# microsoft/esvit

Measured on NVIDIA H100. Metric: multi-crop images/sec, Swin-T W7 pretrain step (2 global 224^2 + 8 local 96^2 crops, DDINOLoss V+R, K=65536), higher is better.
Workload: dtype bf16

## Files before the change

### esvit_b200/_lib.py

```python
from __future__ import annotations

import ctypes
import os
from ctypes import c_double, c_float, c_int, c_longlong, c_void_p

HERE = os.path.dirname(os.path.abspath(__file__))
LIB_PATH = os.path.join(HERE, "lib", "libesvit_b200.so")
HEADER_PATH = os.path.join(os.path.dirname(HERE), "include", "esvit_b200.h")

ERR_BAD_ARG = 1001

P, I, L, F, D = c_void_p, c_int, c_longlong, c_float, c_double

SIGNATURES = {
    "esvit_add_ln_fwd": [P, P, P, I, P, P, F, P, P, I, P, P, L, I, P],
    "esvit_add_ln_bwd": [P, I, P, P, P, P, P, P, I, P, P, P, P, P, L, I, P],
    "esvit_patch_merge_ln_fwd": [P, P, P, F, P, P, P, I, I, I, I, P],
    "esvit_patch_merge_ln_bwd": [P, P, P, P, P, P, P, P, I, I, I, I, P],
    "esvit_token_mean_fwd": [P, P, I, I, I, P],
    "esvit_token_mean_bwd": [P, P, P, I, I, I, P],
    "esvit_patch_embed_fwd": [P, P, P, P, P, F, P, P, P, I, I, I, I, P],
    "esvit_patch_embed_bwd": [P, P, P, P, P, P, P, P, P, P, P, I, I, I, I, P],
    "esvit_window_attn_expand_bias": [P, P, I, I, P],
    "esvit_window_attn_fwd": [P, P, P, P, I, P, P, I, I, I, I, I, I, I, F, P],
    "esvit_window_attn_bwd": [P, P, P, P, I, P, P, P, P, P, P, I, I, I, I, I, I, I, F, P],
    "esvit_window_attn_probs": [P, P, P, P, I, P, I, I, I, I, I, I, I, F, P],
    "esvit_gemm_bias_act": [P, P, P, P, P, L, I, I, I, P],
    "esvit_gemm_mul_colsum": [P, P, P, P, P, P, L, I, I, P],
    "esvit_gemm_bf16": [P, P, P, P, P, L, I, I, I, I, I, I, P],
    "esvit_gemm_mul_colsum2": [P, P, P, P, P, P, L, I, I, I, I, P],
    "esvit_gemm_wgrad_ws_floats": [I, I],
    "esvit_gemm_wgrad": [P, P, P, P, L, I, I, I, I, P],
    "esvit_gelu_fwd": [P, P, L, P],
    "esvit_gelu_bwd": [P, P, P, L, P],
    "esvit_gelu_bwd_dbias": [P, P, P, P, L, I, P],
    "esvit_mul_bwd_dbias": [P, P, P, P, L, I, P],
    "esvit_l2norm_fwd": [P, P, P, F, L, I, P],
    "esvit_l2norm_bwd": [P, P, P, P, L, I, P],
    "esvit_weight_norm_fwd": [P, P, P, P, L, I, P],
    "esvit_weight_norm_bwd": [P, P, P, P, I, P, P, L, I, P],
    "esvit_row_lse": [P, P, F, P, L, I, P],
    "esvit_dino_ce_fwd": [P, P, P, P, P, P, P, F, F, P, L, I, P],
    "esvit_dino_ce_bwd": [P, P, P, P, P, P, P, P, P, F, F, P, L, I, P],
    "esvit_weighted_sum": [P, P, I, P, P],
    "esvit_row_softmax_q_max_k": [],
    "esvit_row_softmax_q": [P, P, F, P, P, L, I, P],
    "esvit_dino_ce_q_fwd": [P, P, P, P, P, F, P, L, I, P],
    "esvit_dino_ce_q_bwd": [P, P, P, P, P, P, P, F, P, L, I, P],
    "esvit_colsum_workspace_rows": [],
    "esvit_colsum": [P, L, I, P, P, P],
    "esvit_center_ema": [P, P, F, F, P, I, P],
    "esvit_normalize_rows": [P, P, L, I, F, P],
    "esvit_region_match": [P, P, I, I, I, I, I, P, P, P],
    "esvit_mhsa_fwd": [P, P, P, I, I, I, I, F, P],
    "esvit_mhsa_bwd": [P, P, P, P, P, P, I, I, I, I, F, P],
    "esvit_vit_patches": [P, P, I, I, I, P],
    "esvit_vit_tokens_fwd": [P, P, P, P, I, I, I, P],
    "esvit_vit_tokens_bwd": [P, P, P, P, P, I, I, I, I, P],
    "esvit_vit_split": [P, P, P, I, I, I, I, P],
    "esvit_ema_multi": [P, P, P, I, D, P],
    "esvit_clip_multi": [P, P, I, F, P, P, P],
    "esvit_grad_sumsq_multi": [P, P, I, P, P],
    "esvit_adamw_ema_multi": [P, P, P, P, P, P, P, P, I, P, P, P, P],
    "esvit_knn_prep": [P, P, P, P, L, L, I, P],
    "esvit_knn_select": [P, L, P, P, P, P, P, I, I, I, I, I, P, P, P, P, P, P],
# ... 29 lines not shown

def _cuda_error_string(code: int) -> str:
    try:
        import torch
        return torch.cuda.cudart().cudaGetErrorString(code) if hasattr(torch.cuda.cudart(), "cudaGetErrorString") \
            else f"cudaError {code}"
    except Exception:
        return f"cudaError {code}"


def call(name: str, *args) -> None:
    rc = getattr(load(), name)(*args)
    if rc != 0:
        if rc == ERR_BAD_ARG:
            raise ValueError(f"{name}: unsupported shape / argument (ESVIT_ERR_BAD_ARG)")
        raise EsvitKernelError(f"{name} failed: {_cuda_error_string(rc)} (status {rc})")


_LAUNCHES = {"esvit_colsum": 2, "esvit_gemm_mul_colsum": 2, "esvit_gemm_mul_colsum2": 2, "esvit_gemm_wgrad": 2}
_launch_count = 0
_timed_names = set()
_timed_events = []
_META = {
    "esvit_dino_ce_bwd": lambda a: {"rows": int(a[-3]), "K": int(a[-2])},
    "esvit_window_attn_bwd": lambda a: _attn_meta(a),
    "esvit_window_attn_fwd": lambda a: _attn_meta(a),
    "esvit_window_attn_probs": lambda a: _attn_meta(a),
    "esvit_gemm_bias_act": lambda a: {"M": int(a[5]), "N": int(a[6]), "K": int(a[7])},
    "esvit_gemm_mul_colsum": lambda a: {"M": int(a[6]), "N": int(a[7]), "K": int(a[8])},
    "esvit_gemm_bf16": lambda a: {"M": int(a[5]), "N": int(a[6]), "K": int(a[7]), "b_mn": int(a[9]), "act": int(a[10]),
                                  "pre": a[4] is not None and a[4].value is not None},
    "esvit_gemm_mul_colsum2": lambda a: {"M": int(a[6]), "N": int(a[7]), "K": int(a[8])},
    "esvit_gemm_wgrad": lambda a: {"T": int(a[4]), "N": int(a[5]), "K": int(a[6])},
    "esvit_add_ln_fwd": lambda a: {"T": int(a[-3]), "C": int(a[-2]), "has_x": a[0] is not None and a[0].value is not None,
                                   "has_delta": a[1] is not None and a[1].value is not None},
    "esvit_add_ln_bwd": lambda a: {"T": int(a[-3]), "C": int(a[-2])},
    "esvit_dino_ce_fwd": lambda a: {"rows": int(a[-3]), "K": int(a[-2])},
    "esvit_dino_ce_q_fwd": lambda a: {"rows": int(a[-3]), "K": int(a[-2])},
    "esvit_dino_ce_q_bwd": lambda a: {"rows": int(a[-3]), "K": int(a[-2])},
    "esvit_row_softmax_q": lambda a: {"rows": int(a[-3]), "K": int(a[-2])},
    "esvit_mhsa_fwd": lambda a: {"B": int(a[3]), "L": int(a[4]), "C": int(a[5]), "nH": int(a[6])},
    "esvit_mhsa_bwd": lambda a: {"B": int(a[6]), "L": int(a[7]), "C": int(a[8]), "nH": int(a[9])},
    "esvit_vit_tokens_bwd": lambda a: {"B": int(a[-5]), "N": int(a[-4]), "D": int(a[-3])},
    "esvit_patch_embed_fwd": lambda a: {"B": int(a[-5]), "H": int(a[-4]), "W": int(a[-3]), "E": int(a[-2])},
    "esvit_patch_embed_bwd": lambda a: {"B": int(a[-5]), "H": int(a[-4]), "W": int(a[-3]), "E": int(a[-2])},
}


def _attn_meta(a):
    B, H, W, C, nH, ws = (int(a[i]) for i in (-9, -8, -7, -6, -5, -4))
    return {"tokens": B * H * W, "C": C, "nH": nH, "ws": ws, "windows": B * (-(-H // ws)) * (-(-W // ws))}


def reset_counters() -> None:
    global _launch_count
    _launch_count = 0
    _timed_events.clear()


def launch_count() -> int:
    return _launch_count


def time_entry_point(names) -> None:
    global _timed_names
    if names is None:
# ... 41 lines not shown
```

### esvit_b200/csrc/gemm2_wgmma.cu

```cuda
#include <cuda.h>

#include "common.cuh"

namespace hg {

constexpr int BK = 64;
constexpr int FOLD_THREADS = 64;
constexpr int SMEM_LIMIT = 232448;
enum { EPI_BIAS = 0, EPI_GELU = 1, EPI_MUL = 2, EPI_F32 = 3 };

__device__ __forceinline__ uint32_t smem_u32(const void* p) { return (uint32_t)__cvta_generic_to_shared(p); }
__device__ __forceinline__ void mbar_init(uint64_t* bar, uint32_t count) {
  asm volatile("mbarrier.init.shared::cta.b64 [%0], %1;\n" ::"r"(smem_u32(bar)), "r"(count));
}
__device__ __forceinline__ void mbar_expect_tx(uint64_t* bar, uint32_t bytes) {
  asm volatile("mbarrier.arrive.expect_tx.shared::cta.b64 _, [%0], %1;\n" ::"r"(smem_u32(bar)), "r"(bytes) : "memory");
}
__device__ __forceinline__ void mbar_arrive(uint64_t* bar) {
  asm volatile("mbarrier.arrive.shared::cta.b64 _, [%0];\n" ::"r"(smem_u32(bar)) : "memory");
}
__device__ __forceinline__ uint64_t global_ns() {
  uint64_t t;
  asm volatile("mov.u64 %0, %%globaltimer;\n" : "=l"(t));
  return t;
// ... 54 lines not shown
  uint64_t d = 0;
  d |= (uint64_t)((smem_addr & 0x3FFFF) >> 4);
  d |= (uint64_t)(mn_major ? (8192 >> 4) : 1) << 16;
  d |= (uint64_t)(1024 >> 4) << 32;
  d |= (uint64_t)1 << 62;
  return d;
}
__device__ __forceinline__ void wgmma_fence() { asm volatile("wgmma.fence.sync.aligned;\n" ::: "memory"); }
__device__ __forceinline__ void wgmma_commit() { asm volatile("wgmma.commit_group.sync.aligned;\n" ::: "memory"); }
template <int N>
__device__ __forceinline__ void wgmma_wait() { asm volatile("wgmma.wait_group.sync.aligned %0;\n" ::"n"(N) : "memory"); }

template <int TA, int TB>
__device__ __forceinline__ void wgmma_n128(float (&d)[64], uint64_t da, uint64_t db, uint32_t scale_d) {
  asm volatile(
      "{\n\t.reg .pred p;\n\t"
      "setp.ne.b32 p, %66, 0;\n\t"
      "wgmma.mma_async.sync.aligned.m64n128k16.f32.bf16.bf16 "
      "{%0, %1, %2, %3, %4, %5, %6, %7, %8, %9, %10, %11, %12, %13, %14, %15, %16, %17, %18, %19, %20, %21, %22, %23, %24, %25, %26, %27, %28, %29, %30, %31, %32, %33, %34, %35, %36, %37, %38, %39, %40, %41, %42, %43, %44, %45, %46, %47, %48, %49, %50, %51, %52, %53, %54, %55, %56, %57, %58, %59, %60, %61, %62, %63}, "
      "%64, %65, p, 1, 1, %67, %68;\n\t}\n"
      : "+f"(d[0]), "+f"(d[1]), "+f"(d[2]), "+f"(d[3]), "+f"(d[4]), "+f"(d[5]), "+f"(d[6]), "+f"(d[7]), "+f"(d[8]), "+f"(d[9]), "+f"(d[10]), "+f"(d[11]), "+f"(d[12]), "+f"(d[13]), "+f"(d[14]), "+f"(d[15]), "+f"(d[16]), "+f"(d[17]), "+f"(d[18]), "+f"(d[19]), "+f"(d[20]), "+f"(d[21]), "+f"(d[22]), "+f"(d[23]), "+f"(d[24]), "+f"(d[25]), "+f"(d[26]), "+f"(d[27]), "+f"(d[28]), "+f"(d[29]), "+f"(d[30]), "+f"(d[31]), "+f"(d[32]), "+f"(d[33]), "+f"(d[34]), "+f"(d[35]), "+f"(d[36]), "+f"(d[37]), "+f"(d[38]), "+f"(d[39]), "+f"(d[40]), "+f"(d[41]), "+f"(d[42]), "+f"(d[43]), "+f"(d[44]), "+f"(d[45]), "+f"(d[46]), "+f"(d[47]), "+f"(d[48]), "+f"(d[49]), "+f"(d[50]), "+f"(d[51]), "+f"(d[52]), "+f"(d[53]), "+f"(d[54]), "+f"(d[55]), "+f"(d[56]), "+f"(d[57]), "+f"(d[58]), "+f"(d[59]), "+f"(d[60]), "+f"(d[61]), "+f"(d[62]), "+f"(d[63])
      : "l"(da), "l"(db), "r"(scale_d), "n"(TA), "n"(TB));
}
template <int TA, int TB>
__device__ __forceinline__ void wgmma_n256(float (&d)[128], uint64_t da, uint64_t db, uint32_t scale_d) {
  asm volatile(
      "{\n\t.reg .pred p;\n\t"
      "setp.ne.b32 p, %130, 0;\n\t"
      "wgmma.mma_async.sync.aligned.m64n256k16.f32.bf16.bf16 "
      "{%0, %1, %2, %3, %4, %5, %6, %7, %8, %9, %10, %11, %12, %13, %14, %15, %16, %17, %18, %19, %20, %21, %22, %23, %24, %25, %26, %27, %28, %29, %30, %31, %32, %33, %34, %35, %36, %37, %38, %39, %40, %41, %42, %43, %44, %45, %46, %47, %48, %49, %50, %51, %52, %53, %54, %55, %56, %57, %58, %59, %60, %61, %62, %63, %64, %65, %66, %67, %68, %69, %70, %71, %72, %73, %74, %75, %76, %77, %78, %79, %80, %81, %82, %83, %84, %85, %86, %87, %88, %89, %90, %91, %92, %93, %94, %95, %96, %97, %98, %99, %100, %101, %102, %103, %104, %105, %106, %107, %108, %109, %110, %111, %112, %113, %114, %115, %116, %117, %118, %119, %120, %121, %122, %123, %124, %125, %126, %127}, "
      "%128, %129, p, 1, 1, %131, %132;\n\t}\n"
      : "+f"(d[0]), "+f"(d[1]), "+f"(d[2]), "+f"(d[3]), "+f"(d[4]), "+f"(d[5]), "+f"(d[6]), "+f"(d[7]), "+f"(d[8]), "+f"(d[9]), "+f"(d[10]), "+f"(d[11]), "+f"(d[12]), "+f"(d[13]), "+f"(d[14]), "+f"(d[15]), "+f"(d[16]), "+f"(d[17]), "+f"(d[18]), "+f"(d[19]), "+f"(d[20]), "+f"(d[21]), "+f"(d[22]), "+f"(d[23]), "+f"(d[24]), "+f"(d[25]), "+f"(d[26]), "+f"(d[27]), "+f"(d[28]), "+f"(d[29]), "+f"(d[30]), "+f"(d[31]), "+f"(d[32]), "+f"(d[33]), "+f"(d[34]), "+f"(d[35]), "+f"(d[36]), "+f"(d[37]), "+f"(d[38]), "+f"(d[39]), "+f"(d[40]), "+f"(d[41]), "+f"(d[42]), "+f"(d[43]), "+f"(d[44]), "+f"(d[45]), "+f"(d[46]), "+f"(d[47]), "+f"(d[48]), "+f"(d[49]), "+f"(d[50]), "+f"(d[51]), "+f"(d[52]), "+f"(d[53]), "+f"(d[54]), "+f"(d[55]), "+f"(d[56]), "+f"(d[57]), "+f"(d[58]), "+f"(d[59]), "+f"(d[60]), "+f"(d[61]), "+f"(d[62]), "+f"(d[63]), "+f"(d[64]), "+f"(d[65]), "+f"(d[66]), "+f"(d[67]), "+f"(d[68]), "+f"(d[69]), "+f"(d[70]), "+f"(d[71]), "+f"(d[72]), "+f"(d[73]), "+f"(d[74]), "+f"(d[75]), "+f"(d[76]), "+f"(d[77]), "+f"(d[78]), "+f"(d[79]), "+f"(d[80]), "+f"(d[81]), "+f"(d[82]), "+f"(d[83]), "+f"(d[84]), "+f"(d[85]), "+f"(d[86]), "+f"(d[87]), "+f"(d[88]), "+f"(d[89]), "+f"(d[90]), "+f"(d[91]), "+f"(d[92]), "+f"(d[93]), "+f"(d[94]), "+f"(d[95]), "+f"(d[96]), "+f"(d[97]), "+f"(d[98]), "+f"(d[99]), "+f"(d[100]), "+f"(d[101]), "+f"(d[102]), "+f"(d[103]), "+f"(d[104]), "+f"(d[105]), "+f"(d[106]), "+f"(d[107]), "+f"(d[108]), "+f"(d[109]), "+f"(d[110]), "+f"(d[111]), "+f"(d[112]), "+f"(d[113]), "+f"(d[114]), "+f"(d[115]), "+f"(d[116]), "+f"(d[117]), "+f"(d[118]), "+f"(d[119]), "+f"(d[120]), "+f"(d[121]), "+f"(d[122]), "+f"(d[123]), "+f"(d[124]), "+f"(d[125]), "+f"(d[126]), "+f"(d[127])
      : "l"(da), "l"(db), "r"(scale_d), "n"(TA), "n"(TB));
}

template <int BN, int TA, int TB>
__device__ __forceinline__ void wgmma_tile(float (&d)[BN / 2], uint64_t da, uint64_t db, uint32_t scale_d) {
  if constexpr (BN == 256) wgmma_n256<TA, TB>(d, da, db, scale_d);
  else wgmma_n128<TA, TB>(d, da, db, scale_d);
}

constexpr float GELU_A = 0.7978845608028654f, GELU_B = 0.7978845608028654f * 0.044715f;
__device__ __forceinline__ float tanh_approx(float x) {
  float y;
  asm("tanh.approx.f32 %0, %1;\n" : "=f"(y) : "f"(x));
  return y;
}
__device__ __forceinline__ float gelu_fwd(float x) {
  const float x2 = x * x;
  const float th = tanh_approx(x * fmaf(GELU_B, x2, GELU_A));
  const float hx = 0.5f * x;
  return fmaf(hx, th, hx);
}
__device__ __forceinline__ float gelu_fwd_grad(float x, float& dy) {
  const float x2 = x * x;
  const float th = tanh_approx(x * fmaf(GELU_B, x2, GELU_A));
  const float hx = 0.5f * x;
  const float m = fmaf(th, th, -1.f);
  const float nc = fmaf(-3.f * GELU_B, x2, -GELU_A);
  dy = fmaf(hx * m, nc, fmaf(0.5f, th, 0.5f));
  return fmaf(hx, th, hx);
}

struct Params {
  const float* bias;
  bf16* out;
// ... 245 lines not shown
            stmatrix_x4(addr, o[0], o[1], o[2], o[3]);
            if constexpr (EPI == EPI_GELU)
              if (p.aux) stmatrix_x4(addr + C::CHUNK_BYTES, d[0], d[1], d[2], d[3]);
          }
        }
        fence_proxy_async();
        if constexpr (EPI != EPI_MUL)
          if (leader) bulk_wait_read<0>();
        named_barrier(1 + wg, 128);
        if (leader) {
          const int gc = n0 + 64 * c, gr = m0 + 64 * wg;
          if (gc < p.N && gr < p.M) {
            tma_store_2d(&map_o, buf, gc, gr);
            if constexpr (EPI == EPI_GELU)
              if (p.aux) tma_store_2d(&map_x, buf + C::CHUNK_BYTES, gc, gr);
          }
          bulk_commit();
          if constexpr (EPI == EPI_MUL) {
            if (c > 0) { bulk_wait_read<1>(); mbar_arrive(&mul_empty[c - 1]); }
            if (c == NCHUNK - 1) { bulk_wait_read<0>(); mbar_arrive(&mul_empty[c]); }
          }
        }
      }
      if constexpr (EPI == EPI_MUL) {
        __syncwarp();
        if (lane == 0) mbar_arrive(cs_full);
      }
    }
    if constexpr (EPI != EPI_F32)
      if (t == 0) bulk_wait_all();
  }
}

typedef CUresult (*EncodeFn)(CUtensorMap*, CUtensorMapDataType, cuuint32_t, void*, const cuuint64_t*, const cuuint64_t*,
                             const cuuint32_t*, const cuuint32_t*, CUtensorMapInterleave, CUtensorMapSwizzle,
                             CUtensorMapL2promotion, CUtensorMapFloatOOBfill);

static EncodeFn get_encode() {
  static EncodeFn fn = nullptr;
  if (!fn) {
    void* ptr = nullptr;
    cudaDriverEntryPointQueryResult qres;
    if (cudaGetDriverEntryPoint("cuTensorMapEncodeTiled", &ptr, cudaEnableDefault, &qres) == cudaSuccess &&
        qres == cudaDriverEntryPointSuccess)
      fn = (EncodeFn)ptr;
  }
  return fn;
}

static bool make_map(CUtensorMap* map, const void* ptr, long long rows, long long cols, int box_rows) {
  EncodeFn enc = get_encode();
  if (!enc) return false;
  cuuint64_t dims[2] = {(cuuint64_t)cols, (cuuint64_t)rows};
  cuuint64_t strides[1] = {(cuuint64_t)cols * 2};
  cuuint32_t box[2] = {64u, (cuuint32_t)box_rows};
  cuuint32_t estr[2] = {1, 1};
  return enc(map, CU_TENSOR_MAP_DATA_TYPE_BFLOAT16, 2, const_cast<void*>(ptr), dims, strides, box, estr,
             CU_TENSOR_MAP_INTERLEAVE_NONE, CU_TENSOR_MAP_SWIZZLE_128B, CU_TENSOR_MAP_L2_PROMOTION_L2_128B,
             CU_TENSOR_MAP_FLOAT_OOB_FILL_NONE) == CUDA_SUCCESS;
}

__global__ void __launch_bounds__(256) colsum_fold_kernel(const float* __restrict__ ws, int rows, int N, float* __restrict__ colsum) {
  const int n = blockIdx.x * 256 + threadIdx.x;
  if (n >= N) return;
  float s = 0.f;
  for (int r = 0; r < rows; r++) s += ws[(long long)r * N + n];
  colsum[n] += s;
}

__global__ void __launch_bounds__(256) split_fold_kernel(const float* __restrict__ part, int splits, long long n4,
                                                         float* __restrict__ out, int accumulate) {
  const long long i = (long long)blockIdx.x * 256 + threadIdx.x;
  if (i >= n4) return;
  float4 s = accumulate ? reinterpret_cast<const float4*>(out)[i] : make_float4(0.f, 0.f, 0.f, 0.f);
  for (int k = 0; k < splits; k++) {
    const float4 t = reinterpret_cast<const float4*>(part)[(long long)k * n4 + i];
    s.x += t.x; s.y += t.y; s.z += t.z; s.w += t.w;
  }
  reinterpret_cast<float4*>(out)[i] = s;
}

constexpr int MAX_GRID = 160;

struct Call {
  const void* a; const void* b;
  int a_mn, b_mn;
  Params p;
};

template <int WG, int BN, int EPI, int AMN, int BMN>
static int launch_cfg(const Call& c, void* stream, int* rows_out) {
  using C = Cfg<WG, BN, EPI>;
// ... 120 lines not shown
ESVIT_API int esvit_gemm_wgrad_ws_floats(int N, int K) {
  const long long n = wgrad_ws_floats(N, K);
  return n > 0x7fffffffLL ? -1 : (int)n;
}
ESVIT_API int esvit_gemm_wgrad(const void* dy, const void* x, float* dw, float* ws, long long T, int N, int K,
                               int accumulate, int tile, void* stream) {
  if (T <= 0 || N <= 0 || K <= 0 || (N % 8) || (K % 8) || T > 0x7fffffffLL || !ws) return ESVIT_ERR_BAD_ARG;
  int wg, bn;
  hg::pick_tile_wgrad(N, K, tile, &wg, &bn);
  const int m_tiles = (N + 64 * wg - 1) / (64 * wg), n_tiles = (K + bn - 1) / bn;
  const int tiles = m_tiles * n_tiles;
  const int k_blocks = (int)((T + hg::BK - 1) / hg::BK);
  const int ctas = esvit_num_sms();
  int splits = tiles >= ctas ? 1 : ctas / tiles;
  if (splits > k_blocks / 8) splits = k_blocks / 8;
  if (tile >= 10000) splits = tile / 10000;
  const long long cap = wgrad_ws_floats(N, K) / ((long long)N * K);
  if (splits > cap) splits = (int)cap;
  if (splits > k_blocks) splits = k_blocks;
  if (splits < 1) splits = 1;
  int kbs = (k_blocks + splits - 1) / splits;
  splits = (k_blocks + kbs - 1) / kbs;
  hg::Call c;
  c.a = dy; c.b = x; c.a_mn = 1; c.b_mn = 1;
  c.p.bias = nullptr; c.p.out = nullptr; c.p.aux = nullptr; c.p.colsum = nullptr; c.p.part = ws;
  c.p.M = N; c.p.N = K; c.p.K = (int)T; c.p.splits = splits; c.p.kb_per_split = kbs;
  const int rc = hg::launch(c, hg::EPI_F32, wg, bn, stream);
  if (rc != 0) return rc;
  const long long n4 = (long long)N * K / 4;
  hg::split_fold_kernel<<<(unsigned)((n4 + 255) / 256), 256, 0, (cudaStream_t)stream>>>(ws, splits, n4, dw, accumulate);
  ESVIT_LAUNCH_CHECK();
}

ESVIT_API int esvit_gemm_bias_act(const void* a, const void* w, const float* bias, void* out, void* pre, long long M,
                                  int N, int K, int act, void* stream) {
  return esvit_gemm_bf16(a, w, bias, out, pre, M, N, K, 0, 0, act, 0, stream);
}
ESVIT_API int esvit_gemm_mul_colsum(const void* a, const void* w, const void* mult, void* out, float* colsum, float* ws,
                                    long long M, int N, int K, void* stream) {
  return esvit_gemm_mul_colsum2(a, w, mult, out, colsum, ws, M, N, K, 0, 0, stream);
}
```

### esvit_b200/linear.py

```python
from __future__ import annotations

from typing import Optional

import torch
from torch.autograd import Function
from torch.autograd.function import once_differentiable

from . import ops

Tensor = torch.Tensor
BF16 = torch.bfloat16
F32 = torch.float32


def _wgrad(key, dy2: Tensor, x2: Tensor, shape):
    d = ops._Arena.accs
    if d is None:
        return ops.gemm_wgrad(dy2, x2).view(shape)
    buf = d.get(key)
    if buf is not None and tuple(buf.shape) == tuple(shape):
        ops.gemm_wgrad(dy2, x2, out=buf, accumulate=True)
        return None
    buf = d[key] = ops.gemm_wgrad(dy2, x2).view(shape)
    return buf.view(shape)


class LinearFn(Function):

    @staticmethod
    def forward(ctx, x, wp, w16, bias):
        y = ops.gemm(x, w16, bias)
        ctx.save_for_backward(x, w16)
        ctx.wkey = ("w", wp.data_ptr())
        ctx.wshape = tuple(wp.shape)
        return y

    @staticmethod
    @once_differentiable
    def backward(ctx, g):
        x, w16 = ctx.saved_tensors
        g = ops._chk(g, BF16, "g")
        N, K = w16.shape
        g2 = g.reshape(-1, N)
        dx = ops.gemm(g2, w16, None, b_mn=True).view(x.shape) if ctx.needs_input_grad[0] else None
        dw = _wgrad(ctx.wkey, g2, x.reshape(-1, K), ctx.wshape) if ctx.needs_input_grad[1] else None
        return dx, dw, None, None


class MlpFn(Function):

    @staticmethod
    def forward(ctx, x, w1p, w1, b1, w2p, w2, b2):
        need = any(ctx.needs_input_grad)
        if need:
            h, pre = ops.gemm(x, w1, b1, act=1, want_pre=True)
        else:
            h, pre = ops.gemm(x, w1, b1, act=1), None
        y = ops.gemm(h, w2, b2)
        ctx.save_for_backward(x, w1, w2, pre, h)
        ctx.keys = (("w", w1p.data_ptr()), tuple(w1p.shape), ("w", w2p.data_ptr()), tuple(w2p.shape))
        ctx.bias_meta = (b1.shape, b1.device, b1.data_ptr())
        return y

    @staticmethod
    @once_differentiable
    def backward(ctx, g):
        x, w1, w2, pre, h = ctx.saved_tensors
        k1, s1, k2, s2 = ctx.keys
        g = ops._chk(g, BF16, "g")
        Cc, Nh = g.shape[-1], pre.shape[-1]
        g2 = g.reshape(-1, Cc)
        dw2 = _wgrad(k2, g2, h.reshape(-1, Nh), s2) if ctx.needs_input_grad[4] else None
        db1, first = ops._acc(("bias", ctx.bias_meta[2]), tuple(ctx.bias_meta[0]), ctx.bias_meta[1])
        dpre = ops.gemm_mul_colsum(g2, w2, pre.reshape(-1, Nh), db1, b_mn=True)
        dx = ops.gemm(dpre, w1, None, b_mn=True).view(x.shape) if ctx.needs_input_grad[0] else None
        dw1 = _wgrad(k1, dpre, x.reshape(-1, x.shape[-1]), s1) if ctx.needs_input_grad[1] else None
        return dx, dw1, None, (db1 if first else None), dw2, None, None


class HeadMlpFn(Function):

    @staticmethod
    def forward(ctx, x, w1p, w1, b1, w2p, w2, b2, w3p, w3, b3):
        need = any(ctx.needs_input_grad)
        if need:
            h1, p1 = ops.gemm(x, w1, b1, act=1, want_pre=True)
            h2, p2 = ops.gemm(h1, w2, b2, act=1, want_pre=True)
        else:
            h1, p1 = ops.gemm(x, w1, b1, act=1), None
            h2, p2 = ops.gemm(h1, w2, b2, act=1), None
        y = ops.gemm(h2, w3, b3)
# ... 43 lines not shown
```

### esvit_b200/ops.py

```python
from __future__ import annotations

import ctypes
from typing import List, Optional, Sequence, Tuple

import torch
from torch.autograd import Function
from torch.autograd.function import once_differentiable

from . import _lib, shadow

Tensor = torch.Tensor
BF16 = torch.bfloat16
F32 = torch.float32


def _p(t: Optional[Tensor]):
    return ctypes.c_void_p(t.data_ptr()) if t is not None else None


def _po(t: Tensor, off_elems: int):
    return ctypes.c_void_p(t.data_ptr() + off_elems * t.element_size())


def _stream():
# ... 721 lines not shown

def gemm(a: Tensor, b: Tensor, bias: Optional[Tensor] = None, act: int = 0, want_pre: bool = False, a_mn: bool = False,
         b_mn: bool = False, tile: int = 0):
    a, b = _chk(a, BF16, "a"), _chk(b, BF16, "b")
    bias = _chk(bias, F32, "bias")
    if a_mn:
        K, M = a.shape
        lead = (M,)
    else:
        K = a.shape[-1]
        M = a.numel() // K
        lead = tuple(a.shape[:-1])
    N = b.shape[1] if b_mn else b.shape[0]
    assert (b.shape[0] if b_mn else b.shape[1]) == K, (a.shape, b.shape)
    out = torch.empty(*lead, N, dtype=BF16, device=a.device)
    pre = torch.empty_like(out) if (act and want_pre) else None
    _lib.call("esvit_gemm_bf16", _p(a), _p(b), _p(bias), _p(out), _p(pre), M, N, K, 1 if a_mn else 0, 1 if b_mn else 0, act,
              tile, _stream())
    return (out, pre) if (act and want_pre) else out


def gemm_mul_colsum(a: Tensor, b: Tensor, mult: Tensor, colsum: Tensor, b_mn: bool = False, tile: int = 0) -> Tensor:
    a, b, mult = _chk(a, BF16, "a"), _chk(b, BF16, "b"), _chk(mult, BF16, "mult")
    K = a.shape[-1]
    M = a.numel() // K
    N = b.shape[1] if b_mn else b.shape[0]
    out = torch.empty_like(mult)
    ws = torch.empty(GEMM_COLSUM_WS_ROWS * N, dtype=F32, device=a.device)
    _lib.call("esvit_gemm_mul_colsum2", _p(a), _p(b), _p(mult), _p(out), _p(colsum), _p(ws), M, N, K, 1 if b_mn else 0, tile,
              _stream())
    return out


_wgrad_ws = {}


def gemm_wgrad(dy: Tensor, x: Tensor, out: Optional[Tensor] = None, accumulate: bool = False, tile: int = 0) -> Tensor:
    dy, x = _chk(dy, BF16, "dy"), _chk(x, BF16, "x")
    N, K = dy.shape[-1], x.shape[-1]
    T = dy.numel() // N
    assert x.numel() // K == T
    if out is None:
        out = torch.empty(N, K, dtype=F32, device=dy.device)
        accumulate = False
    key = (dy.device, N, K)
    ws = _wgrad_ws.get(key)
    if ws is None:
        n = _lib.load().esvit_gemm_wgrad_ws_floats(N, K)
        if n <= 0:
            raise ValueError("esvit_gemm_wgrad: weight too large for the split-K workspace")
        ws = _wgrad_ws[key] = torch.empty(n, dtype=F32, device=dy.device)
    _lib.call("esvit_gemm_wgrad", _p(dy), _p(x), _p(out), _p(ws), T, N, K, 1 if accumulate else 0, tile, _stream())
    return out


class LinearGeluFn(Function):

    @staticmethod
    def forward(ctx, x, w, bias):
        out, pre = gemm_bias_act(x, w, bias, act=1, want_pre=True)
        ctx.save_for_backward(x, w, pre)
        ctx.bias_meta = (bias.shape, bias.device, bias.data_ptr())
        return out

    @staticmethod
    @once_differentiable
# ... 263 lines not shown
```

### include/esvit_b200.h

```cpp
#ifndef ESVIT_B200_H
#define ESVIT_B200_H

#ifdef __cplusplus
extern "C" {
#endif

#define ESVIT_ERR_BAD_ARG 1001

int esvit_add_ln_fwd(const float* x, const void* delta, const float* keep, int tokens_per_sample,
                     const float* gamma, const float* beta, float eps, float* xout, void* y, int y_is_bf16,
                     float* mean, float* rstd, long long T, int C, void* stream);
int esvit_add_ln_bwd(const void* dy, int dy_is_bf16, const float* dxo, const float* xs, const float* mean,
                     const float* rstd, const float* gamma, const float* keep, int tokens_per_sample, float* dx,
                     void* ddelta, float* dgamma, float* dbeta, float* ddelta_bias, long long T, int C, void* stream);

int esvit_patch_merge_ln_fwd(const float* x, const float* gamma, const float* beta, float eps, void* y, float* mean,
                             float* rstd, int B, int H, int W, int C, void* stream);
int esvit_patch_merge_ln_bwd(const void* dy, const float* x, const float* mean, const float* rstd,
                             const float* gamma, float* dx, float* dgamma, float* dbeta, int B, int H, int W, int C,
                             void* stream);

int esvit_token_mean_fwd(const float* region, float* pooled, int B, int N, int C, void* stream);
int esvit_token_mean_bwd(const float* dpooled, const float* dregion_in, float* dregion, int B, int N, int C,
                         void* stream);

int esvit_patch_embed_fwd(const float* img, const float* w, const float* bias, const float* gamma, const float* beta,
                          float eps, float* out, float* mean, float* rstd, int B, int H, int W, int E, void* stream);
int esvit_patch_embed_bwd(const float* img, const float* w, const float* bias, const float* gamma, const float* mean,
                          const float* rstd, const float* dout, float* dw, float* dbias, float* dgamma, float* dbeta,
                          int B, int H, int W, int E, void* stream);

int esvit_window_attn_expand_bias(const float* bias_table, float* bias_ws, int nH, int ws, void* stream);
int esvit_window_attn_fwd(const void* qkv, const void* qkv_bias, const float* bias_table, float* bias_ws, int bias_ready,
                          void* out, float* lse, int B, int H, int W, int C, int nH, int ws, int shift, float scale,
                          void* stream);
int esvit_window_attn_bwd(const void* qkv, const void* qkv_bias, const float* bias_table, float* bias_ws, int bias_ready,
                          const void* out, const void* dout, const float* lse, void* dqkv, float* dbias_table,
                          float* dqkv_bias, int B, int H, int W, int C, int nH, int ws, int shift, float scale,
                          void* stream);
int esvit_window_attn_probs(const void* qkv, const void* qkv_bias, const float* bias_table, float* bias_ws, int bias_ready,
                            float* probs, int B, int H, int W, int C, int nH, int ws, int shift, float scale, void* stream);

int esvit_gemm_bias_act(const void* a, const void* w, const float* bias, void* out, void* pre, long long M, int N, int K,
                        int act, void* stream);
int esvit_gemm_mul_colsum(const void* a, const void* w, const void* mult, void* out, float* colsum, float* ws,
                          long long M, int N, int K, void* stream);

int esvit_gemm_bf16(const void* a, const void* b, const float* bias, void* out, void* pre, long long M, int N, int K,
                    int a_mn, int b_mn, int act, int tile, void* stream);
int esvit_gemm_mul_colsum2(const void* a, const void* b, const void* mult, void* out, float* colsum, float* ws,
                           long long M, int N, int K, int b_mn, int tile, void* stream);
int esvit_gemm_wgrad_ws_floats(int N, int K);
int esvit_gemm_wgrad(const void* dy, const void* x, float* dw, float* ws, long long T, int N, int K, int accumulate,
                     int tile, void* stream);

int esvit_gelu_fwd(const void* x, void* y, long long n, void* stream);
int esvit_gelu_bwd(const void* x, const void* dy, void* dx, long long n, void* stream);
int esvit_gelu_bwd_dbias(const void* x, const void* dy, void* dx, float* dbias, long long R, int N, void* stream);
int esvit_mul_bwd_dbias(const void* gp, const void* dy, void* dx, float* dbias, long long R, int N, void* stream);

int esvit_l2norm_fwd(const void* x, void* y, float* inv, float eps, long long R, int D, void* stream);
int esvit_l2norm_bwd(const void* x, const void* dy, const float* inv, void* dx, long long R, int D, void* stream);
int esvit_weight_norm_fwd(const float* v, const float* g, void* w, float* norm, long long K, int D, void* stream);
int esvit_weight_norm_bwd(const float* v, const float* g, const float* norm, const void* dw, int dw_is_f32, float* dv,
                          float* dg, long long K, int D, void* stream);

int esvit_row_lse(const void* x, const float* center, float inv_temp, float* lse, long long R, int K, void* stream);
int esvit_dino_ce_fwd(const void* s, const void* t, const float* center, float* lse_s, const float* lse_t,
                      const int* trow, const int* order, float inv_temp_t, float inv_tau_s, float* row_loss, long long R,
                      int K, void* stream);
int esvit_dino_ce_bwd(const void* s, const void* t, const float* center, const float* lse_s, const float* lse_t,
                      const int* trow, const int* order, const float* w, const float* gscale, float inv_temp_t,
                      float inv_tau_s, void* ds, long long R, int K, void* stream);
int esvit_weighted_sum(const float* v, const float* w, int R, float* out, void* stream);
int esvit_row_softmax_q_max_k(void);
int esvit_row_softmax_q(const void* x, const float* center, float inv_temp, float* lse, void* q, long long R, int K,
                        void* stream);
int esvit_dino_ce_q_fwd(const void* s, const void* q, float* lse_s, const int* trow, const int* order, float inv_tau_s,
                        float* row_loss, long long R, int K, void* stream);
int esvit_dino_ce_q_bwd(const void* s, const void* q, const float* lse_s, const int* trow, const int* order,
                        const float* w, const float* gscale, float inv_tau_s, void* ds, long long R, int K, void* stream);

int esvit_colsum_workspace_rows(void);
int esvit_colsum(const void* t, long long R, int K, float* workspace, float* out, void* stream);
int esvit_center_ema(const float* center, const float* colsum, float rows_total, float momentum, float* center_out,
                     int K, void* stream);

// ... 43 lines not shown
```

Measured before the change: 1006.

## Fuse Swin MLP fc1+GELU+fc2 forward into one warp-specialized WGMMA kernel

Adds a persistent Hopper kernel that computes fc1, bias, GELU and fc2 in one pass for C in {96,128,192}. It keeps each 64-wide hidden chunk in registers and feeds it to the second GEMM as a register-sourced WGMMA operand, with TMA weight streaming through an mbarrier ring and a dedicated producer warpgroup. This removes the round trip of the 4C hidden activation through global memory on the teacher path. On the student path it still writes h and the GELU gradient for backward. The cost is lower occupancy (one CTA of 384 threads per SM), heavy register pressure, and C=768 stages falling back to the old path.

```diff
diff --git a/esvit_b200/_lib.py b/esvit_b200/_lib.py
--- a/esvit_b200/_lib.py
+++ b/esvit_b200/_lib.py
@@ -31,6 +31,7 @@
     "esvit_gemm_mul_colsum2": [P, P, P, P, P, P, L, I, I, I, I, P],
     "esvit_gemm_wgrad_ws_floats": [I, I],
     "esvit_gemm_wgrad": [P, P, P, P, L, I, I, I, I, P],
+    "esvit_mlp_fwd": [P, P, P, P, P, P, P, P, L, I, P],
     "esvit_gelu_fwd": [P, P, L, P],
     "esvit_gelu_bwd": [P, P, P, L, P],
     "esvit_gelu_bwd_dbias": [P, P, P, P, L, I, P],
@@ -126,6 +127,7 @@
                                   "pre": a[4] is not None and a[4].value is not None},
     "esvit_gemm_mul_colsum2": lambda a: {"M": int(a[6]), "N": int(a[7]), "K": int(a[8])},
     "esvit_gemm_wgrad": lambda a: {"T": int(a[4]), "N": int(a[5]), "K": int(a[6])},
+    "esvit_mlp_fwd": lambda a: {"M": int(a[8]), "C": int(a[9]), "student": a[6] is not None and a[6].value is not None},
     "esvit_add_ln_fwd": lambda a: {"T": int(a[-3]), "C": int(a[-2]), "has_x": a[0] is not None and a[0].value is not None,
                                    "has_delta": a[1] is not None and a[1].value is not None},
     "esvit_add_ln_bwd": lambda a: {"T": int(a[-3]), "C": int(a[-2])},
diff --git a/esvit_b200/csrc/gemm2_wgmma.cu b/esvit_b200/csrc/gemm2_wgmma.cu
--- a/esvit_b200/csrc/gemm2_wgmma.cu
+++ b/esvit_b200/csrc/gemm2_wgmma.cu
@@ -110,6 +110,47 @@
       "%128, %129, p, 1, 1, %131, %132;\n\t}\n"
       : "+f"(d[0]), "+f"(d[1]), "+f"(d[2]), "+f"(d[3]), "+f"(d[4]), "+f"(d[5]), "+f"(d[6]), "+f"(d[7]), "+f"(d[8]), "+f"(d[9]), "+f"(d[10]), "+f"(d[11]), "+f"(d[12]), "+f"(d[13]), "+f"(d[14]), "+f"(d[15]), "+f"(d[16]), "+f"(d[17]), "+f"(d[18]), "+f"(d[19]), "+f"(d[20]), "+f"(d[21]), "+f"(d[22]), "+f"(d[23]), "+f"(d[24]), "+f"(d[25]), "+f"(d[26]), "+f"(d[27]), "+f"(d[28]), "+f"(d[29]), "+f"(d[30]), "+f"(d[31]), "+f"(d[32]), "+f"(d[33]), "+f"(d[34]), "+f"(d[35]), "+f"(d[36]), "+f"(d[37]), "+f"(d[38]), "+f"(d[39]), "+f"(d[40]), "+f"(d[41]), "+f"(d[42]), "+f"(d[43]), "+f"(d[44]), "+f"(d[45]), "+f"(d[46]), "+f"(d[47]), "+f"(d[48]), "+f"(d[49]), "+f"(d[50]), "+f"(d[51]), "+f"(d[52]), "+f"(d[53]), "+f"(d[54]), "+f"(d[55]), "+f"(d[56]), "+f"(d[57]), "+f"(d[58]), "+f"(d[59]), "+f"(d[60]), "+f"(d[61]), "+f"(d[62]), "+f"(d[63]), "+f"(d[64]), "+f"(d[65]), "+f"(d[66]), "+f"(d[67]), "+f"(d[68]), "+f"(d[69]), "+f"(d[70]), "+f"(d[71]), "+f"(d[72]), "+f"(d[73]), "+f"(d[74]), "+f"(d[75]), "+f"(d[76]), "+f"(d[77]), "+f"(d[78]), "+f"(d[79]), "+f"(d[80]), "+f"(d[81]), "+f"(d[82]), "+f"(d[83]), "+f"(d[84]), "+f"(d[85]), "+f"(d[86]), "+f"(d[87]), "+f"(d[88]), "+f"(d[89]), "+f"(d[90]), "+f"(d[91]), "+f"(d[92]), "+f"(d[93]), "+f"(d[94]), "+f"(d[95]), "+f"(d[96]), "+f"(d[97]), "+f"(d[98]), "+f"(d[99]), "+f"(d[100]), "+f"(d[101]), "+f"(d[102]), "+f"(d[103]), "+f"(d[104]), "+f"(d[105]), "+f"(d[106]), "+f"(d[107]), "+f"(d[108]), "+f"(d[109]), "+f"(d[110]), "+f"(d[111]), "+f"(d[112]), "+f"(d[113]), "+f"(d[114]), "+f"(d[115]), "+f"(d[116]), "+f"(d[117]), "+f"(d[118]), "+f"(d[119]), "+f"(d[120]), "+f"(d[121]), "+f"(d[122]), "+f"(d[123]), "+f"(d[124]), "+f"(d[125]), "+f"(d[126]), "+f"(d[127])
       : "l"(da), "l"(db), "r"(scale_d), "n"(TA), "n"(TB));
+}
+
+__device__ __forceinline__ void wgmma_ss_n64(float (&d)[32], uint64_t da, uint64_t db, uint32_t scale_d) {
+  asm volatile(
+      "{\n\t.reg .pred p;\n\t"
+      "setp.ne.b32 p, %34, 0;\n\t"
+      "wgmma.mma_async.sync.aligned.m64n64k16.f32.bf16.bf16 "
+      "{%0, %1, %2, %3, %4, %5, %6, %7, %8, %9, %10, %11, %12, %13, %14, %15, %16, %17, %18, %19, %20, %21, %22, %23, %24, %25, %26, %27, %28, %29, %30, %31}, "
+      "%32, %33, p, 1, 1, 0, 0;\n\t}\n"
+      : "+f"(d[0]), "+f"(d[1]), "+f"(d[2]), "+f"(d[3]), "+f"(d[4]), "+f"(d[5]), "+f"(d[6]), "+f"(d[7]), "+f"(d[8]), "+f"(d[9]), "+f"(d[10]), "+f"(d[11]), "+f"(d[12]), "+f"(d[13]), "+f"(d[14]), "+f"(d[15]), "+f"(d[16]), "+f"(d[17]), "+f"(d[18]), "+f"(d[19]), "+f"(d[20]), "+f"(d[21]), "+f"(d[22]), "+f"(d[23]), "+f"(d[24]), "+f"(d[25]), "+f"(d[26]), "+f"(d[27]), "+f"(d[28]), "+f"(d[29]), "+f"(d[30]), "+f"(d[31])
+      : "l"(da), "l"(db), "r"(scale_d));
+}
+__device__ __forceinline__ void wgmma_rs(float (&d)[48], const uint32_t (&a)[4], uint64_t db, uint32_t scale_d) {
+  asm volatile(
+      "{\n\t.reg .pred p;\n\t"
+      "setp.ne.b32 p, %53, 0;\n\t"
+      "wgmma.mma_async.sync.aligned.m64n96k16.f32.bf16.bf16 "
+      "{%0, %1, %2, %3, %4, %5, %6, %7, %8, %9, %10, %11, %12, %13, %14, %15, %16, %17, %18, %19, %20, %21, %22, %23, %24, %25, %26, %27, %28, %29, %30, %31, %32, %33, %34, %35, %36, %37, %38, %39, %40, %41, %42, %43, %44, %45, %46, %47}, "
+      "{%48, %49, %50, %51}, %52, p, 1, 1, 0;\n\t}\n"
+      : "+f"(d[0]), "+f"(d[1]), "+f"(d[2]), "+f"(d[3]), "+f"(d[4]), "+f"(d[5]), "+f"(d[6]), "+f"(d[7]), "+f"(d[8]), "+f"(d[9]), "+f"(d[10]), "+f"(d[11]), "+f"(d[12]), "+f"(d[13]), "+f"(d[14]), "+f"(d[15]), "+f"(d[16]), "+f"(d[17]), "+f"(d[18]), "+f"(d[19]), "+f"(d[20]), "+f"(d[21]), "+f"(d[22]), "+f"(d[23]), "+f"(d[24]), "+f"(d[25]), "+f"(d[26]), "+f"(d[27]), "+f"(d[28]), "+f"(d[29]), "+f"(d[30]), "+f"(d[31]), "+f"(d[32]), "+f"(d[33]), "+f"(d[34]), "+f"(d[35]), "+f"(d[36]), "+f"(d[37]), "+f"(d[38]), "+f"(d[39]), "+f"(d[40]), "+f"(d[41]), "+f"(d[42]), "+f"(d[43]), "+f"(d[44]), "+f"(d[45]), "+f"(d[46]), "+f"(d[47])
+      : "r"(a[0]), "r"(a[1]), "r"(a[2]), "r"(a[3]), "l"(db), "r"(scale_d));
+}
+__device__ __forceinline__ void wgmma_rs(float (&d)[64], const uint32_t (&a)[4], uint64_t db, uint32_t scale_d) {
+  asm volatile(
+      "{\n\t.reg .pred p;\n\t"
+      "setp.ne.b32 p, %69, 0;\n\t"
+      "wgmma.mma_async.sync.aligned.m64n128k16.f32.bf16.bf16 "
+      "{%0, %1, %2, %3, %4, %5, %6, %7, %8, %9, %10, %11, %12, %13, %14, %15, %16, %17, %18, %19, %20, %21, %22, %23, %24, %25, %26, %27, %28, %29, %30, %31, %32, %33, %34, %35, %36, %37, %38, %39, %40, %41, %42, %43, %44, %45, %46, %47, %48, %49, %50, %51, %52, %53, %54, %55, %56, %57, %58, %59, %60, %61, %62, %63}, "
+      "{%64, %65, %66, %67}, %68, p, 1, 1, 0;\n\t}\n"
+      : "+f"(d[0]), "+f"(d[1]), "+f"(d[2]), "+f"(d[3]), "+f"(d[4]), "+f"(d[5]), "+f"(d[6]), "+f"(d[7]), "+f"(d[8]), "+f"(d[9]), "+f"(d[10]), "+f"(d[11]), "+f"(d[12]), "+f"(d[13]), "+f"(d[14]), "+f"(d[15]), "+f"(d[16]), "+f"(d[17]), "+f"(d[18]), "+f"(d[19]), "+f"(d[20]), "+f"(d[21]), "+f"(d[22]), "+f"(d[23]), "+f"(d[24]), "+f"(d[25]), "+f"(d[26]), "+f"(d[27]), "+f"(d[28]), "+f"(d[29]), "+f"(d[30]), "+f"(d[31]), "+f"(d[32]), "+f"(d[33]), "+f"(d[34]), "+f"(d[35]), "+f"(d[36]), "+f"(d[37]), "+f"(d[38]), "+f"(d[39]), "+f"(d[40]), "+f"(d[41]), "+f"(d[42]), "+f"(d[43]), "+f"(d[44]), "+f"(d[45]), "+f"(d[46]), "+f"(d[47]), "+f"(d[48]), "+f"(d[49]), "+f"(d[50]), "+f"(d[51]), "+f"(d[52]), "+f"(d[53]), "+f"(d[54]), "+f"(d[55]), "+f"(d[56]), "+f"(d[57]), "+f"(d[58]), "+f"(d[59]), "+f"(d[60]), "+f"(d[61]), "+f"(d[62]), "+f"(d[63])
+      : "r"(a[0]), "r"(a[1]), "r"(a[2]), "r"(a[3]), "l"(db), "r"(scale_d));
+}
+__device__ __forceinline__ void wgmma_rs(float (&d)[96], const uint32_t (&a)[4], uint64_t db, uint32_t scale_d) {
+  asm volatile(
+      "{\n\t.reg .pred p;\n\t"
+      "setp.ne.b32 p, %101, 0;\n\t"
+      "wgmma.mma_async.sync.aligned.m64n192k16.f32.bf16.bf16 "
+      "{%0, %1, %2, %3, %4, %5, %6, %7, %8, %9, %10, %11, %12, %13, %14, %15, %16, %17, %18, %19, %20, %21, %22, %23, %24, %25, %26, %27, %28, %29, %30, %31, %32, %33, %34, %35, %36, %37, %38, %39, %40, %41, %42, %43, %44, %45, %46, %47, %48, %49, %50, %51, %52, %53, %54, %55, %56, %57, %58, %59, %60, %61, %62, %63, %64, %65, %66, %67, %68, %69, %70, %71, %72, %73, %74, %75, %76, %77, %78, %79, %80, %81, %82, %83, %84, %85, %86, %87, %88, %89, %90, %91, %92, %93, %94, %95}, "
+      "{%96, %97, %98, %99}, %100, p, 1, 1, 0;\n\t}\n"
+      : "+f"(d[0]), "+f"(d[1]), "+f"(d[2]), "+f"(d[3]), "+f"(d[4]), "+f"(d[5]), "+f"(d[6]), "+f"(d[7]), "+f"(d[8]), "+f"(d[9]), "+f"(d[10]), "+f"(d[11]), "+f"(d[12]), "+f"(d[13]), "+f"(d[14]), "+f"(d[15]), "+f"(d[16]), "+f"(d[17]), "+f"(d[18]), "+f"(d[19]), "+f"(d[20]), "+f"(d[21]), "+f"(d[22]), "+f"(d[23]), "+f"(d[24]), "+f"(d[25]), "+f"(d[26]), "+f"(d[27]), "+f"(d[28]), "+f"(d[29]), "+f"(d[30]), "+f"(d[31]), "+f"(d[32]), "+f"(d[33]), "+f"(d[34]), "+f"(d[35]), "+f"(d[36]), "+f"(d[37]), "+f"(d[38]), "+f"(d[39]), "+f"(d[40]), "+f"(d[41]), "+f"(d[42]), "+f"(d[43]), "+f"(d[44]), "+f"(d[45]), "+f"(d[46]), "+f"(d[47]), "+f"(d[48]), "+f"(d[49]), "+f"(d[50]), "+f"(d[51]), "+f"(d[52]), "+f"(d[53]), "+f"(d[54]), "+f"(d[55]), "+f"(d[56]), "+f"(d[57]), "+f"(d[58]), "+f"(d[59]), "+f"(d[60]), "+f"(d[61]), "+f"(d[62]), "+f"(d[63]), "+f"(d[64]), "+f"(d[65]), "+f"(d[66]), "+f"(d[67]), "+f"(d[68]), "+f"(d[69]), "+f"(d[70]), "+f"(d[71]), "+f"(d[72]), "+f"(d[73]), "+f"(d[74]), "+f"(d[75]), "+f"(d[76]), "+f"(d[77]), "+f"(d[78]), "+f"(d[79]), "+f"(d[80]), "+f"(d[81]), "+f"(d[82]), "+f"(d[83]), "+f"(d[84]), "+f"(d[85]), "+f"(d[86]), "+f"(d[87]), "+f"(d[88]), "+f"(d[89]), "+f"(d[90]), "+f"(d[91]), "+f"(d[92]), "+f"(d[93]), "+f"(d[94]), "+f"(d[95])
+      : "r"(a[0]), "r"(a[1]), "r"(a[2]), "r"(a[3]), "l"(db), "r"(scale_d));
 }
 
 template <int BN, int TA, int TB>
@@ -421,6 +462,207 @@
   }
 }
 
+template <int C>
+struct MlpCfg {
+  static constexpr int BM = 128, HB = 64;
+  static constexpr int KB = (C + 63) / 64;
+  static constexpr int NH = 4 * C / HB;
+  static constexpr int X_BYTES = KB * BM * 128;
+  static constexpr int W1_BYTES = KB * HB * 128;
+  static constexpr int W2_BYTES = C * 128;
+  static constexpr int STAGE_BYTES = W1_BYTES + W2_BYTES;
+  static constexpr int CHUNK_BYTES = BM * 128;
+  static constexpr int EP_BYTES = 2 * CHUNK_BYTES;
+  static constexpr int BAR_BYTES = 128;
+  static constexpr int STAGES_RAW = (SMEM_LIMIT - 1024 - BAR_BYTES - 2 * X_BYTES - EP_BYTES) / STAGE_BYTES;
+  static constexpr int STAGES = STAGES_RAW > 4 ? 4 : STAGES_RAW;
+  static constexpr int SMEM = 1024 + 2 * X_BYTES + STAGES * STAGE_BYTES + EP_BYTES + BAR_BYTES;
+  static_assert(C % 32 == 0 && C <= 192, "acc2 [64 x C] must fit the consumer registers; C / 8 even");
+  static_assert(STAGES >= 2, "weight ring too shallow");
+  static_assert(SMEM <= SMEM_LIMIT, "shared memory budget");
+  static_assert((2 * STAGES + 4) * 8 <= BAR_BYTES, "mbarrier area");
+};
+
+struct MlpParams {
+  const float* b1;
+  const float* b2;
+  int M;
+};
+
+template <int C, bool STORE>
+__global__ void __launch_bounds__(384, 1) mlp_fwd_kernel(const __grid_constant__ CUtensorMap map_x,
+                                                         const __grid_constant__ CUtensorMap map_w1,
+                                                         const __grid_constant__ CUtensorMap map_w2,
+                                                         const __grid_constant__ CUtensorMap map_y,
+                                                         const __grid_constant__ CUtensorMap map_h,
+                                                         const __grid_constant__ CUtensorMap map_g, const MlpParams p) {
+  using G = MlpCfg<C>;
+  constexpr int BM = G::BM, KB = G::KB, NH = G::NH, STAGES = G::STAGES;
+  extern __shared__ __align__(1024) uint8_t smem_raw[];
+  uint8_t* xs = smem_raw + ((1024u - (smem_u32(smem_raw) & 1023u)) & 1023u);
+  uint8_t* ws = xs + 2 * G::X_BYTES;
+  uint8_t* ep = ws + STAGES * G::STAGE_BYTES;
+  uint64_t* full = reinterpret_cast<uint64_t*>(ep + G::EP_BYTES);
+  uint64_t* empty = full + STAGES;
+  uint64_t* x_full = empty + STAGES;
+  uint64_t* x_empty = x_full + 2;
+
+  const int wg = threadIdx.x >> 7;
+  const int num_items = (p.M + BM - 1) / BM;
+  if (threadIdx.x == 0) {
+    asm volatile("prefetch.tensormap [%0];\n" ::"l"(&map_x) : "memory");
+    asm volatile("prefetch.tensormap [%0];\n" ::"l"(&map_w1) : "memory");
+    asm volatile("prefetch.tensormap [%0];\n" ::"l"(&map_w2) : "memory");
+    for (int i = 0; i < STAGES; i++) { mbar_init(&full[i], 1); mbar_init(&empty[i], 256); }
+    for (int i = 0; i < 2; i++) { mbar_init(&x_full[i], 1); mbar_init(&x_empty[i], 256); }
+    asm volatile("fence.mbarrier_init.release.cluster;\n" ::: "memory");
+  }
+  __syncthreads();
+
+  if (wg == 2) {
+    asm volatile("setmaxnreg.dec.sync.aligned.u32 40;\n" ::: "memory");
+    if (threadIdx.x == 256) {
+      int stage = 0;
+      uint32_t phase = 0;
+      int local = 0;
+      for (int item = blockIdx.x; item < num_items; item += gridDim.x, local++) {
+        const int m0 = item * BM, xb = local & 1;
+        mbar_wait(&x_empty[xb], ((local >> 1) & 1) ^ 1);
+        mbar_expect_tx(&x_full[xb], G::X_BYTES);
+#pragma unroll
+        for (int kb = 0; kb < KB; kb++)
+          tma_load_2d(smem_u32(xs + xb * G::X_BYTES + kb * BM * 128), &map_x, &x_full[xb], kb * 64, m0);
+        for (int j = 0; j < NH; j++) {
+          mbar_wait(&empty[stage], phase ^ 1);
+          const uint32_t sw = smem_u32(ws + stage * G::STAGE_BYTES);
+          mbar_expect_tx(&full[stage], G::STAGE_BYTES);
+#pragma unroll
+          for (int kb = 0; kb < KB; kb++) tma_load_2d(sw + kb * 8192, &map_w1, &full[stage], kb * 64, j * 64);
+          tma_load_2d(sw + G::W1_BYTES, &map_w2, &full[stage], j * 64, 0);
+          if (++stage == STAGES) { stage = 0; phase ^= 1; }
+        }
+      }
+    }
+  } else {
+    asm volatile("setmaxnreg.inc.sync.aligned.u32 232;\n" ::: "memory");
+    const int t = threadIdx.x & 127, warp = t >> 5, lane = t & 31;
+    const int frag_col = 2 * (lane & 3);
+    const uint32_t lrow = (uint32_t)(warp * 16 + (lane & 15)) * 128u, lsw = lane & 7, lblk = lane >> 4;
+    const bool leader = t == 0;
+    const uint32_t hbuf = smem_u32(ep) + wg * 8192;
+    int stage = 0;
+    uint32_t phase = 0;
+    int local = 0;
+    for (int item = blockIdx.x; item < num_items; item += gridDim.x, local++) {
+      const int m0 = item * BM, xb = local & 1;
+      const uint64_t da = make_smem_desc(smem_u32(xs + xb * G::X_BYTES) + wg * 8192, false);
+      float acc1[32], acc2[C / 2];
+      mbar_wait(&x_full[xb], (local >> 1) & 1);
+      for (int j = 0; j < NH; j++) {
+        {
+          const uint64_t db = make_smem_desc(smem_u32(ws + stage * G::STAGE_BYTES), false);
+          mbar_wait(&full[stage], phase);
+          wgmma_fence();
+#pragma unroll
+          for (int k = 0; k < C / 16; k++)
+            wgmma_ss_n64(acc1, da + (k >> 2) * (BM * 128 >> 4) + (k & 3) * 2, db + (k >> 2) * (8192 >> 4) + (k & 3) * 2,
+                         k ? 1u : 0u);
+          wgmma_commit();
+        }
+        wgmma_wait<0>();
+        if (j == NH - 1) mbar_arrive(&x_empty[xb]);
+        if constexpr (STORE) {
+          if (leader) bulk_wait_read<0>();
+          named_barrier(1 + wg, 128);
+        }
+        uint32_t af[4][4];
+#pragma unroll
+        for (int s = 0; s < 4; s++) {
+          const float* a0 = acc1 + 8 * s;
+          float b[4] = {0.f, 0.f, 0.f, 0.f};
+          if (p.b1) {
+#pragma unroll
+            for (int u = 0; u < 2; u++) {
+              const float2 bb = __ldg(reinterpret_cast<const float2*>(p.b1 + j * 64 + (2 * s + u) * 8 + frag_col));
+              b[2 * u] = bb.x; b[2 * u + 1] = bb.y;
+            }
+          }
+          uint32_t d[4];
+#pragma unroll
+          for (int q = 0; q < 4; q++) {
+            const float v0 = a0[2 * q] + b[2 * (q >> 1)], v1 = a0[2 * q + 1] + b[2 * (q >> 1) + 1];
+            if constexpr (STORE) {
+              float d0, d1;
+              const float y0 = gelu_fwd_grad(v0, d0), y1 = gelu_fwd_grad(v1, d1);
+              af[s][q] = pack_bf162(y0, y1);
+              d[q] = pack_bf162(d0, d1);
+            } else {
+              af[s][q] = pack_bf162(gelu_fwd(v0), gelu_fwd(v1));
+            }
+          }
+          if constexpr (STORE) {
+            const uint32_t addr = hbuf + lrow + (((2 * s + lblk) ^ lsw) << 4);
+            stmatrix_x4(addr, af[s][0], af[s][1], af[s][2], af[s][3]);
+            stmatrix_x4(addr + G::CHUNK_BYTES, d[0], d[1], d[2], d[3]);
+          }
+        }
+        if constexpr (STORE) fence_proxy_async();
+        const uint64_t d2 = make_smem_desc(smem_u32(ws + stage * G::STAGE_BYTES) + G::W1_BYTES, false);
+        wgmma_fence();
+#pragma unroll
+        for (int s = 0; s < 4; s++) wgmma_rs(acc2, af[s], d2 + s * 2, (j > 0 || s > 0) ? 1u : 0u);
+        wgmma_commit();
+        if constexpr (STORE) {
+          named_barrier(1 + wg, 128);
+          if (leader) {
+            const int gr = m0 + 64 * wg;
+            if (gr < p.M) {
+              tma_store_2d(&map_h, hbuf, j * 64, gr);
+              tma_store_2d(&map_g, hbuf + G::CHUNK_BYTES, j * 64, gr);
+            }
+            bulk_commit();
+          }
+        }
+        wgmma_wait<0>();
+        mbar_arrive(&empty[stage]);
+        if (++stage == STAGES) { stage = 0; phase ^= 1; }
+      }
+#pragma unroll
+      for (int c = 0; c < KB; c++) {
+        const uint32_t buf = smem_u32(ep + (c & 1) * G::CHUNK_BYTES) + wg * 8192;
+        if (leader) bulk_wait_read<0>();
+        named_barrier(1 + wg, 128);
+#pragma unroll
+        for (int jj = 0; jj < 8; jj += 2) {
+          const int i = c * 8 + jj;
+          if (i >= C / 8) continue;
+          const float* a0 = acc2 + 4 * i;
+          float b[4] = {0.f, 0.f, 0.f, 0.f};
+          if (p.b2) {
+#pragma unroll
+            for (int u = 0; u < 2; u++) {
+              const float2 bb = __ldg(reinterpret_cast<const float2*>(p.b2 + (i + u) * 8 + frag_col));
+              b[2 * u] = bb.x; b[2 * u + 1] = bb.y;
+            }
+          }
+          uint32_t o[4];
+#pragma unroll
+          for (int q = 0; q < 4; q++) o[q] = pack_bf162(a0[2 * q] + b[2 * (q >> 1)], a0[2 * q + 1] + b[2 * (q >> 1) + 1]);
+          stmatrix_x4(buf + lrow + (((jj + lblk) ^ lsw) << 4), o[0], o[1], o[2], o[3]);
+        }
+        fence_proxy_async();
+        named_barrier(1 + wg, 128);
+        if (leader) {
+          const int gr = m0 + 64 * wg;
+          if (gr < p.M) tma_store_2d(&map_y, buf, c * 64, gr);
+          bulk_commit();
+        }
+      }
+    }
+    if (t == 0) bulk_wait_all();
+  }
+}
+
 typedef CUresult (*EncodeFn)(CUtensorMap*, CUtensorMapDataType, cuuint32_t, void*, const cuuint64_t*, const cuuint64_t*,
                              const cuuint32_t*, const cuuint32_t*, CUtensorMapInterleave, CUtensorMapSwizzle,
                              CUtensorMapL2promotion, CUtensorMapFloatOOBfill);
@@ -447,6 +689,38 @@
   return enc(map, CU_TENSOR_MAP_DATA_TYPE_BFLOAT16, 2, const_cast<void*>(ptr), dims, strides, box, estr,
              CU_TENSOR_MAP_INTERLEAVE_NONE, CU_TENSOR_MAP_SWIZZLE_128B, CU_TENSOR_MAP_L2_PROMOTION_L2_128B,
              CU_TENSOR_MAP_FLOAT_OOB_FILL_NONE) == CUDA_SUCCESS;
+}
+
+template <int C, bool STORE>
+static int mlp_launch(const void* x, const void* w1, const float* b1, const void* w2, const float* b2, void* y, void* h,
+                      void* g, int M, void* stream) {
+  using G = MlpCfg<C>;
+  CUtensorMap mx, m1, m2, my, mh = {}, mg = {};
+  if (!make_map(&mx, x, M, C, G::BM) || !make_map(&m1, w1, 4 * C, C, 64) || !make_map(&m2, w2, C, 4 * C, C) ||
+      !make_map(&my, y, M, C, 64))
+    return ESVIT_ERR_BAD_ARG;
+  if (STORE && (!make_map(&mh, h, M, 4 * C, 64) || !make_map(&mg, g, M, 4 * C, 64))) return ESVIT_ERR_BAD_ARG;
+  auto kernel = mlp_fwd_kernel<C, STORE>;
+  static bool attr_set = false;
+  if (!attr_set) {
+    cudaError_t e = cudaFuncSetAttribute(kernel, cudaFuncAttributeMaxDynamicSharedMemorySize, G::SMEM);
+    if (e != cudaSuccess) return (int)e;
+    attr_set = true;
+  }
+  const int items = (M + G::BM - 1) / G::BM;
+  int grid = esvit_num_sms();
+  if (grid > items) grid = items;
+  MlpParams p;
+  p.b1 = b1; p.b2 = b2; p.M = M;
+  kernel<<<grid, 384, G::SMEM, (cudaStream_t)stream>>>(mx, m1, m2, my, mh, mg, p);
+  return (int)cudaGetLastError();
+}
+
+template <int C>
+static int mlp_launch_c(const void* x, const void* w1, const float* b1, const void* w2, const float* b2, void* y, void* h,
+                        void* g, int M, void* stream) {
+  return h ? mlp_launch<C, true>(x, w1, b1, w2, b2, y, h, g, M, stream)
+           : mlp_launch<C, false>(x, w1, b1, w2, b2, y, h, g, M, stream);
 }
 
 __global__ void __launch_bounds__(256) colsum_fold_kernel(const float* __restrict__ ws, int rows, int N, float* __restrict__ colsum) {
@@ -633,6 +907,21 @@
   ESVIT_LAUNCH_CHECK();
 }
 
+ESVIT_API int esvit_mlp_fwd(const void* x, const void* w1, const float* b1, const void* w2, const float* b2, void* y,
+                            void* h, void* gelu_grad, long long M, int C, void* stream) {
+  auto aligned = [](const void* q, uintptr_t a) { return ((uintptr_t)q & (a - 1)) == 0; };
+  if (M <= 0 || M > 0x7fffffffLL || !x || !w1 || !w2 || !y || (h == nullptr) != (gelu_grad == nullptr)) return ESVIT_ERR_BAD_ARG;
+  if (!aligned(x, 16) || !aligned(w1, 16) || !aligned(w2, 16) || !aligned(y, 16) || !aligned(h, 16) ||
+      !aligned(gelu_grad, 16) || !aligned(b1, 8) || !aligned(b2, 8))
+    return ESVIT_ERR_BAD_ARG;
+  switch (C) {
+    case 96: return hg::mlp_launch_c<96>(x, w1, b1, w2, b2, y, h, gelu_grad, (int)M, stream);
+    case 128: return hg::mlp_launch_c<128>(x, w1, b1, w2, b2, y, h, gelu_grad, (int)M, stream);
+    case 192: return hg::mlp_launch_c<192>(x, w1, b1, w2, b2, y, h, gelu_grad, (int)M, stream);
+  }
+  return ESVIT_ERR_BAD_ARG;
+}
+
 ESVIT_API int esvit_gemm_bias_act(const void* a, const void* w, const float* bias, void* out, void* pre, long long M,
                                   int N, int K, int act, void* stream) {
   return esvit_gemm_bf16(a, w, bias, out, pre, M, N, K, 0, 0, act, 0, stream);
diff --git a/esvit_b200/linear.py b/esvit_b200/linear.py
--- a/esvit_b200/linear.py
+++ b/esvit_b200/linear.py
@@ -52,11 +52,18 @@
     @staticmethod
     def forward(ctx, x, w1p, w1, b1, w2p, w2, b2):
         need = any(ctx.needs_input_grad)
-        if need:
-            h, pre = ops.gemm(x, w1, b1, act=1, want_pre=True)
+        C = x.shape[-1]
+        if C in ops.MLP_FUSED_C and w1.shape[0] == 4 * C:
+            if need:
+                y, h, pre = ops.mlp_fwd(x, w1, b1, w2, b2, want_h=True)
+            else:
+                y, h, pre = ops.mlp_fwd(x, w1, b1, w2, b2), None, None
         else:
-            h, pre = ops.gemm(x, w1, b1, act=1), None
-        y = ops.gemm(h, w2, b2)
+            if need:
+                h, pre = ops.gemm(x, w1, b1, act=1, want_pre=True)
+            else:
+                h, pre = ops.gemm(x, w1, b1, act=1), None
+            y = ops.gemm(h, w2, b2)
         ctx.save_for_backward(x, w1, w2, pre, h)
         ctx.keys = (("w", w1p.data_ptr()), tuple(w1p.shape), ("w", w2p.data_ptr()), tuple(w2p.shape))
         ctx.bias_meta = (b1.shape, b1.device, b1.data_ptr())
diff --git a/esvit_b200/ops.py b/esvit_b200/ops.py
--- a/esvit_b200/ops.py
+++ b/esvit_b200/ops.py
@@ -777,6 +777,22 @@
     return out
 
 
+MLP_FUSED_C = (96, 128, 192)
+
+
+def mlp_fwd(x: Tensor, w1: Tensor, b1: Optional[Tensor], w2: Tensor, b2: Optional[Tensor], want_h: bool = False):
+    x, w1, w2 = _chk(x, BF16, "x"), _chk(w1, BF16, "w1"), _chk(w2, BF16, "w2")
+    b1, b2 = _chk(b1, F32, "b1"), _chk(b2, F32, "b2")
+    C = x.shape[-1]
+    M = x.numel() // C
+    assert tuple(w1.shape) == (4 * C, C) and tuple(w2.shape) == (C, 4 * C), (x.shape, w1.shape, w2.shape)
+    y = torch.empty_like(x)
+    h = torch.empty(*x.shape[:-1], 4 * C, dtype=BF16, device=x.device) if want_h else None
+    pre = torch.empty_like(h) if want_h else None
+    _lib.call("esvit_mlp_fwd", _p(x), _p(w1), _p(b1), _p(w2), _p(b2), _p(y), _p(h), _p(pre), M, C, _stream())
+    return (y, h, pre) if want_h else y
+
+
 _wgrad_ws = {}
 
 
diff --git a/include/esvit_b200.h b/include/esvit_b200.h
--- a/include/esvit_b200.h
+++ b/include/esvit_b200.h
@@ -53,6 +53,8 @@
 int esvit_gemm_wgrad_ws_floats(int N, int K);
 int esvit_gemm_wgrad(const void* dy, const void* x, float* dw, float* ws, long long T, int N, int K, int accumulate,
                      int tile, void* stream);
+int esvit_mlp_fwd(const void* x, const void* w1, const float* b1, const void* w2, const float* b2, void* y, void* h,
+                  void* gelu_grad, long long M, int C, void* stream);
 
 int esvit_gelu_fwd(const void* x, void* y, long long n, void* stream);
 int esvit_gelu_bwd(const void* x, const void* dy, void* dx, long long n, void* stream);
```

Measured after the change: 1038 (median of 6 runs). 1.03x the previous value.
